# cmaestre/pcl_tracking

Hardware: AMD Instinct MI355X
Metric: particles x input-points / sec per frame (tracked frames/sec @8192 particles per GPU) (higher is better)
Workload: dtype f32

## Files before the change

pcl_tracking_amd/build.py:

```python
import os
import subprocess
import sys

_HERE = os.path.dirname(os.path.abspath(__file__))
CSRC = os.path.join(_HERE, "csrc")
OUT_DIR = os.path.join(_HERE, "_build")
LIB = os.path.join(OUT_DIR, "libpft_hip.so")
SOURCES = ["pft_kernels.hip", "pft_octree.hip", "pft_octree_gated.hip", "pft_octree_sorted.hip", "pft_likelihood.hip", "pft_population.hip", "pft_kld.hip", "pft_change.hip", "pft_exact_nn.hip", "pft_hull.hip", "pft_api.hip", "pft_frame.hip", "pft_api_debug.hip", "pft_api_features.hip",
           "pft_filters.hip", "pft_segment.hip", "pft_report.hip", "pft_model.hip", "pft_match.hip", "pft_reacquire.hip", "pft_spread.hip", "pft_refine.hip", "pft_subtract.hip", "pft_visibility.hip", "pft_depth.hip", "pft_grow.hip", "pft_view.hip"]
HEADERS = ["pft_internal.h", "pft_tracker.h", "pft_devbuf.h", "pft_device_utils.h", "pft_vis_project.h", "pft_alias.h", "pft_octree_box.h", "pft_report_solve.h", "pft_match_search.h", "pft_pair_tree.h", "pft_spread_final.h", "pft_refine_solve.h", "pft_segment_solve.h", os.path.join("..", "..", "include", "pft.h"),
           os.path.join("..", "..", "include", "pft_filters.h"), os.path.join("..", "..", "include", "pft_segment.h"),
           os.path.join("..", "..", "include", "pft_model.h"), os.path.join("..", "..", "include", "pft_subtract.h"),
           os.path.join("..", "..", "include", "pft_visibility.h"), os.path.join("..", "..", "include", "pft_grow.h"),
           os.path.join("..", "..", "include", "pft_view.h")]

HIPCC_FLAGS = [
    "--offload-arch=gfx950", "-O3", "-std=c++17", "-fPIC", "-shared", "-ffp-contract=off",
    "-fno-slp-vectorize",
    "-fno-fast-math", "-Wall", "-Wno-unused-function", "-Wno-unused-value", "-Wno-unused-result",
]


def hipcc():
    for c in (os.environ.get("HIPCC"), "/opt/rocm/bin/hipcc", "hipcc"):
        if c and (os.path.isabs(c) and os.path.exists(c) or not os.path.isabs(c)):
            return c
    return "hipcc"


def needs_build():
    if not os.path.exists(LIB):
        return True
    t = os.path.getmtime(LIB)
    deps = [os.path.join(CSRC, s) for s in SOURCES + HEADERS] + [os.path.abspath(__file__)]
    return any(os.path.getmtime(d) > t for d in deps)


def build(force=False, verbose=False, extra_flags=()):
    extra_flags = list(extra_flags) + os.environ.get("PFT_EXTRA_HIPCC_FLAGS", "").split()
    if not force and not needs_build():
        return LIB
    os.makedirs(OUT_DIR, exist_ok=True)
    cmd = [hipcc()] + HIPCC_FLAGS + list(extra_flags) + ["-o", LIB] + [os.path.join(CSRC, s) for s in SOURCES]
    if verbose:
        print(" ".join(cmd), flush=True)
    r = subprocess.run(cmd, capture_output=True, text=True)
    if r.returncode != 0:
        sys.stderr.write(r.stdout + r.stderr)
        raise RuntimeError("hipcc failed")
    if verbose and (r.stdout or r.stderr):
        print(r.stdout + r.stderr)
    return LIB


EXAMPLES_DIR = os.path.join(_HERE, "examples")
EXAMPLE_BIN = os.path.join(OUT_DIR, "auto_tracking_amd")
DIST_EXAMPLE_BIN = os.path.join(OUT_DIR, "dist_tracking_amd")
CREATE_MODEL_BIN = os.path.join(OUT_DIR, "create_model_amd")
_EXAMPLE_DEPS = [os.path.join(EXAMPLES_DIR, "tracking_app.hpp")] + [
    os.path.join(_HERE, "include", "pft", h) for h in ("particle_filter_tracker.hpp", "filters.hpp", "pcd_io.hpp", "common.hpp", "id_exchange.hpp", "segmentation.hpp", "model_preparation.hpp", "scene_subtraction.hpp", "model_growth.hpp", "pnm_io.hpp")] + [
    os.path.join(EXAMPLES_DIR, "segment_options.hpp")]


def _build_host_program(src, out, extra, force, verbose):
    lib = build()
    deps = [src, lib] + _EXAMPLE_DEPS
    if not force and os.path.exists(out) and all(os.path.getmtime(d) <= os.path.getmtime(out) for d in deps):
        return out
    root = os.path.dirname(_HERE)
    cmd = [hipcc(), "-std=c++17", "-O2", "-Wall", "-ffp-contract=off", "-I", os.path.join(root, "include"),
           "-I", os.path.join(_HERE, "include"), src, "-o", out, "-L", OUT_DIR, "-lpft_hip", "-Wl,-rpath,$ORIGIN"] + extra
    if verbose:
        print(" ".join(cmd), flush=True)
    r = subprocess.run(cmd, capture_output=True, text=True)
    if r.returncode != 0:
        sys.stderr.write(r.stdout + r.stderr)
        raise RuntimeError("example build failed: " + os.path.basename(src))
    return out


def build_host_program(src, out, force=False, verbose=False):
    return _build_host_program(src, out, [], force, verbose)


def build_example(force=False, verbose=False):
    return _build_host_program(os.path.join(EXAMPLES_DIR, "auto_tracking_amd.cpp"), EXAMPLE_BIN, [], force, verbose)


def build_dist_example(force=False, verbose=False):
    rocm = os.environ.get("ROCM_PATH", "/opt/rocm")
    extra = ["-I", os.path.join(rocm, "include"), "-L", os.path.join(rocm, "lib"), "-lrccl", "-lpthread",
             "-Wl,-rpath," + os.path.join(rocm, "lib")]
    return _build_host_program(os.path.join(EXAMPLES_DIR, "dist_tracking_amd.cpp"), DIST_EXAMPLE_BIN, extra, force, verbose)


def build_create_model_example(force=False, verbose=False):
    return _build_host_program(os.path.join(EXAMPLES_DIR, "create_model_amd.cpp"), CREATE_MODEL_BIN, [], force, verbose)


if __name__ == "__main__":
    print(build(force="--force" in sys.argv, verbose=True))
    print(build_example(force="--force" in sys.argv, verbose=True))
    print(build_dist_example(force="--force" in sys.argv, verbose=True))
    print(build_create_model_example(force="--force" in sys.argv, verbose=True))
```

pcl_tracking_amd/csrc/pft_octree.hip:

```cpp
#include "pft_device_utils.h"

#ifdef PFT_DIAG
#define STAMP(k) do { if (threadIdx.x == 0) d.hdr->ticks[k] = wall_clock64(); } while (0)
#define TICK_NOW() wall_clock64()
#else
#define STAMP(k) do { } while (0)
#define TICK_NOW() 0ull
#endif

#include "pft_octree_box.h"

#define PFT_REPLAY_HEAD 1024u
__device__ __forceinline__ void box_replay(BuildSh& S, const float4* __restrict__ pts, uint32_t n, double res, unsigned long long* hdr_ticks) {
  const uint32_t tid = threadIdx.x, nt = blockDim.x;
  const uint32_t head = n < PFT_REPLAY_HEAD ? n : PFT_REPLAY_HEAD;
  float lmn[3] = {FLT_MAX, FLT_MAX, FLT_MAX}, lmx[3] = {-FLT_MAX, -FLT_MAX, -FLT_MAX};
  const uint32_t wt = tid - WAVE, ws = nt - WAVE;
  auto local_aabb = [&]() {
    for (uint32_t i0 = PFT_REPLAY_HEAD + wt; i0 < n; i0 += 8u * ws) {
      float4 q[8];
#pragma unroll
      for (uint32_t k = 0; k < 8u; k++) q[k] = pts[min(i0 + k * ws, n - 1u)];
#pragma unroll
      for (uint32_t k = 0; k < 8u; k++) {
        lmn[0] = fminf(lmn[0], q[k].x); lmx[0] = fmaxf(lmx[0], q[k].x);
        lmn[1] = fminf(lmn[1], q[k].y); lmx[1] = fmaxf(lmx[1], q[k].y);
        lmn[2] = fminf(lmn[2], q[k].z); lmx[2] = fmaxf(lmx[2], q[k].z);
      }
    }
  };
  if (tid >= WAVE) local_aabb();
#ifdef PFT_DIAG
  if (tid == WAVE) hdr_ticks[13] = wall_clock64();
#endif
  if (tid < WAVE) {
    float4 q[PFT_REPLAY_HEAD / WAVE];
#pragma unroll
    for (uint32_t c = 0; c < PFT_REPLAY_HEAD / WAVE; c++) q[c] = pts[min(c * WAVE + tid, n - 1u)];
    uint32_t cur = 1;
    bool stop = false;
    double mn[3] = {S.mn[0], S.mn[1], S.mn[2]}, mx[3] = {S.mx[0], S.mx[1], S.mx[2]};
    int depth = S.depth, ngrow = S.ngrow;
    uint32_t err = S.err;
    const double epsd = (double)FLT_EPSILON;
#pragma unroll
    for (uint32_t c = 0; c < PFT_REPLAY_HEAD / WAVE; c++) {
      const uint32_t gi = c * WAVE + tid;
      const float4 p = q[c];
      while (!stop) {
        const bool viol = gi >= cur && gi < head && box_violates(p.x, p.y, p.z, mn, mx);
        const unsigned long long bal = __ballot(viol);
        if (!bal) break;
        const int f = __ffsll((long long)bal) - 1;
        const float px = __shfl(p.x, f), py = __shfl(p.y, f), pz = __shfl(p.z, f);
        const uint32_t idx = c * WAVE + (uint32_t)f;
        for (;;) {
          const bool lx = px < mn[0], ly = py < mn[1], lz = pz < mn[2];
          const bool ux = px >= mx[0], uy = py >= mx[1], uz = pz >= mx[2];
          if (!(lx || ly || lz || ux || uy || uz)) break;
          if (ngrow >= PFT_MAX_GROW || depth >= PFT_MAX_DEPTH) {
            err |= 2u;
            break;
          }
          double side = (double)(1u << depth) * res;
          if (tid == 0) {
            S.gidx[ngrow] = idx;
            S.gshift[ngrow] = (ux ? 0u : 1u) | (uy ? 0u : 2u) | (uz ? 0u : 4u);
            S.gold[ngrow] = (uint32_t)depth;
          }
          if (!ux) mn[0] -= side;
          if (!uy) mn[1] -= side;
          if (!uz) mn[2] -= side;
          depth++;
          side = (double)(1u << depth) * res - epsd;
          mx[0] = mn[0] + side;
          mx[1] = mn[1] + side;
          mx[2] = mn[2] + side;
          if (tid == 0) {
            S.gmin[ngrow + 1][0] = mn[0];
            S.gmin[ngrow + 1][1] = mn[1];
            S.gmin[ngrow + 1][2] = mn[2];
          }
          ngrow++;
        }
        cur = idx + 1u;
        if (err) stop = true;
      }
    }
    if (tid == 0) {
      for (int a = 0; a < 3; a++) {
        S.mn[a] = mn[a];
        S.mx[a] = mx[a];
      }
      S.depth = depth;
      S.ngrow = ngrow;
      S.err = err;
    }
    if (tid == 0) S.cur = head;
#ifdef PFT_DIAG
    if (tid == 0) hdr_ticks[14] = wall_clock64();
#endif
  }
  __syncthreads();
  if (S.err || n <= PFT_REPLAY_HEAD) return;
  for (;;) {
    const uint32_t cur = S.cur;
    const double mn[3] = {S.mn[0], S.mn[1], S.mn[2]};
    const double mx[3] = {S.mx[0], S.mx[1], S.mx[2]};
    uint32_t first = 0xffffffffu;
    if (tid >= WAVE && (box_violates(lmn[0], lmn[1], lmn[2], mn, mx) || box_violates(lmx[0], lmx[1], lmx[2], mn, mx))) {
      uint32_t i0 = PFT_REPLAY_HEAD + wt;
      if (i0 < cur) i0 += ((cur - i0 + ws - 1) / ws) * ws;
      for (uint32_t i = i0; i < n; i += ws) {
        const float4 p = pts[i];
        if (box_violates(p.x, p.y, p.z, mn, mx)) {
          first = i;
          break;
        }
      }
    }
    first = block_reduce<uint32_t>(first, S.u32s, OpMinU(), 0xffffffffu);
    if (first == 0xffffffffu) break;
    if (tid == 0) {
      box_grow(S, pts[first], first, res);
      S.cur = first + 1;
    }
    __syncthreads();
    if (S.err) break;
  }
}

template <int K>
struct RegStore {
  typedef uint32_t key_t;
  static constexpr int B = 10;
  static constexpr bool MORTON = true;
  static constexpr uint32_t CODE = K == 4 ? 1u : (K == 8 ? 2u : 3u);
  uint32_t key[K], node[K];
  __device__ RegStore(const PftDev&) {}
  template <class F>
  __device__ __forceinline__ void each(uint32_t n, F&& f) {
#pragma unroll
    for (int j = 0; j < K; j++) {
      uint32_t i = threadIdx.x + j * PFT_BUILD_THREADS;
      if (i < n) f(i, key[j], node[j]);
      UNROLL_FENCE(j, 2);
    }
  }
};

template <int K>
struct HybridStore {
  typedef uint32_t key_t;
  static constexpr int B = 10;
  static constexpr bool MORTON = true;
  static constexpr uint32_t CODE = 4u;
  uint32_t key[K], node[K];
  uint32_t* gkey;
  uint32_t* gnode;
  __device__ HybridStore(const PftDev& d) : gkey(reinterpret_cast<uint32_t*>(d.pt_key64)), gnode(d.pt_node) {}
  template <class F>
  __device__ __forceinline__ void each(uint32_t n, F&& f) {
#pragma unroll
    for (int j = 0; j < K; j++) {
      uint32_t i = threadIdx.x + j * PFT_BUILD_THREADS;
      if (i < n) f(i, key[j], node[j]);
      UNROLL_FENCE(j, 2);
    }
    for (uint32_t i = K * PFT_BUILD_THREADS + threadIdx.x; i < n; i += PFT_BUILD_THREADS) f(i, gkey[i], gnode[i]);
  }
};

struct GlobStore {
  typedef unsigned long long key_t;
  static constexpr int B = 21;
  static constexpr bool MORTON = false;
  static constexpr uint32_t CODE = 5u;
  unsigned long long* key;
  uint32_t* node;
  __device__ GlobStore(const PftDev& d) : key(d.pt_key64), node(d.pt_node) {}
  template <class F>
  __device__ __forceinline__ void each(uint32_t n, F&& f) {
#pragma unroll 4
    for (uint32_t i = threadIdx.x; i < n; i += blockDim.x) f(i, key[i], node[i]);
  }
};

template <class KT, int B, bool MORTON>
__device__ __forceinline__ uint32_t key_child(KT k, int bit) {
  if (MORTON) return (uint32_t)(k >> (3 * bit)) & 7u;
  return (uint32_t)(((k >> (2 * B + bit)) & 1) << 2) | (uint32_t)(((k >> (B + bit)) & 1) << 1) |
         (uint32_t)((k >> bit) & 1);
}

__device__ __forceinline__ uint32_t spread3_10(uint32_t x) {
  x = (x | (x << 16)) & 0x030000FFu;
  x = (x | (x << 8)) & 0x0300F00Fu;
  x = (x | (x << 4)) & 0x030C30C3u;
  x = (x | (x << 2)) & 0x09249249u;
  return x;
}

template <class Store, bool LDSW, bool TMPLDS>
__device__ __forceinline__ bool build_tree(const PftParams& prm, const PftDev& d, BuildSh& S, uint32_t n, uint32_t* lds_words,
                           uint32_t lds_words_cap, uint32_t* lds_tmp, uint32_t* out_leaf_start,
                           uint32_t* out_n_leaves) {
  typedef typename Store::key_t key_t;
  constexpr int B = Store::B;
  const uint32_t tid = threadIdx.x, nt = blockDim.x;
  const float4* pts = d.crop_pts;
  const double res = prm.res, inv_res = 1.0 / prm.res;
  const int D = S.depth, ngrow = S.ngrow;
  Store st(d);
  const int J = (D >= 4 && D <= PFT_TABLE_MAX_DEPTH) ? (D - 1 < PFT_JUMP_MAX_LEVEL ? D - 1 : PFT_JUMP_MAX_LEVEL) : 0;
  if (J > 0) {
    for (uint32_t i = tid; i < 128u; i += nt) S.dn_bits[J][i] = 0u;
    __syncthreads();
  }

  const uint32_t last_grow = ngrow > 0 ? S.gidx[ngrow - 1] : 0u;
  st.each(n, [&](uint32_t i, key_t& key, uint32_t& node) {
    float4 p = pts[i];
    int e = ngrow;
    if (ngrow > 0 && i < last_grow) {
      e = 0;
      while (e < ngrow && S.gidx[e] <= i) e++;
    }
    const double tq[3] = {(double)p.x - S.gmin[e][0], (double)p.y - S.gmin[e][1], (double)p.z - S.gmin[e][2]};
    uint32_t kk[3];
#pragma unroll
    for (int a = 0; a < 3; a++) {
      double q0 = tq[a] * inv_res;
      const double fr = q0 - floor(q0);
      if (fr < 1.0e-6 || fr > 1.0 - 1.0e-6) q0 = tq[a] / res;
      kk[a] = (uint32_t)q0;
    }
    uint32_t kx = kk[0], ky = kk[1], kz = kk[2];
    for (int s = e; s < ngrow; s++) {
      uint32_t sh = S.gshift[s], od = S.gold[s];
      if (sh & 1u) kx += 1u << od;
      if (sh & 2u) ky += 1u << od;
      if (sh & 4u) kz += 1u << od;
    }
    if (d.pt_key) {
      d.pt_key[3 * (size_t)i + 0] = kx;
      d.pt_key[3 * (size_t)i + 1] = ky;
      d.pt_key[3 * (size_t)i + 2] = kz;
    }
    if (Store::MORTON)
      key = (key_t)((spread3_10(kx) << 2) | (spread3_10(ky) << 1) | spread3_10(kz));
    else
      key = ((key_t)kx << (2 * B)) | ((key_t)ky << B) | (key_t)kz;
    node = 0;
  });

  STAMP(2);
  uint32_t* W = LDSW ? lds_words : d.words;
  if (tid == 0) S.jump = J;
  int l0 = 0;
  if (J > 0) {
    uint32_t (*dn_bits)[128] = S.dn_bits;
    uint32_t (*dn_pref)[128] = S.dn_pref;
    uint32_t* dn_cnt = S.dn_cnt;
    st.each(n, [&](uint32_t, key_t& key, uint32_t& node) {
      uint32_t mj = 0;
      if (Store::MORTON)
        mj = (uint32_t)(key >> (3 * (D - J)));
      else
        for (int l = 0; l < J; l++) mj = (mj << 3) | key_child<key_t, B, Store::MORTON>(key, D - 1 - l);
      node = mj;
      const uint32_t bt = 1u << (mj & 31u);
      if (!(dn_bits[J][mj >> 5] & bt)) atomicOr(&dn_bits[J][mj >> 5], bt);
    });
    __syncthreads();
    for (int l = J - 1; l >= 0; l--) {
      const uint32_t nbits = 1u << (3 * l);
      const bool pred = tid < nbits && ((dn_bits[l + 1][tid >> 2] >> (8u * (tid & 3u))) & 0xffu) != 0u;
      const unsigned long long m = __ballot(pred);
      if (lane_id() == 0 && (uint32_t)wave_id() * 64u < ((nbits + 63u) & ~63u)) {
        dn_bits[l][2 * wave_id()] = (uint32_t)m;
        dn_bits[l][2 * wave_id() + 1] = (uint32_t)(m >> 32);
      }
      __syncthreads();
    }
    if (wave_id() <= J) {
      const int l = wave_id(), ln = lane_id();
      const uint32_t nwords = ((1u << (3 * l)) + 31u) >> 5;
      const uint32_t c0 = (uint32_t)ln < nwords ? __popc(dn_bits[l][ln]) : 0u;
      const uint32_t c1 = (uint32_t)ln + 64u < nwords ? __popc(dn_bits[l][ln + 64]) : 0u;
      const uint32_t i0 = wave_incl_scan(c0);
      const uint32_t t0 = (uint32_t)__shfl((int)i0, 63);
      const uint32_t i1 = wave_incl_scan(c1);
      dn_pref[l][ln] = i0 - c0;
      dn_pref[l][ln + 64] = t0 + i1 - c1;
      if (ln == 63) dn_cnt[l] = t0 + i1;
    }
    __syncthreads();
    if (tid == 0) {
      S.lvl[0] = 0;
      for (int l = 0; l <= J; l++) S.lvl[l + 1] = S.lvl[l] + dn_cnt[l];
    }
    __syncthreads();
    const uint32_t top_end = S.lvl[J + 1];
    if (LDSW && top_end + 2 > lds_words_cap) return false;
    if (top_end + 2 > d.max_words) {
      if (tid == 0) S.err |= 1u;
    } else {
#define DN_RANK(l, i) (dn_pref[l][(i) >> 5] + __popc(dn_bits[l][(i) >> 5] & ((1u << ((i) & 31u)) - 1u)))
      for (uint32_t cand = tid; cand < 585u; cand += nt) {
        int l = 0;
        uint32_t i = cand;
        while (l < J && i >= (1u << (3 * l))) {
          i -= 1u << (3 * l);
          l++;
        }
        if (l < J && ((dn_bits[l][i >> 5] >> (i & 31u)) & 1u)) {
          const uint32_t mask = (dn_bits[l + 1][i >> 2] >> (8u * (i & 3u))) & 0xffu;
          const uint32_t base = S.lvl[l + 1] + DN_RANK(l + 1, 8u * i);
          W[S.lvl[l] + DN_RANK(l, i)] = mask | (base << 8);
        }
      }
      for (uint32_t j = S.lvl[J] + tid; j < top_end; j += nt) W[j] = 0;
      for (uint32_t i = tid; i < (1u << (3 * J)); i += nt) {
        uint32_t cx = 0, cy = 0, cz = 0;
        for (int b = 0; b < J; b++) {
          const uint32_t dg = (i >> (3 * b)) & 7u;
          cx |= (dg >> 2) << b;
          cy |= ((dg >> 1) & 1u) << b;
          cz |= (dg & 1u) << b;
        }
        const bool occ = (dn_bits[J][i >> 5] >> (i & 31u)) & 1u;
        d.jump[cx | (cy << J) | (cz << (2 * J))] = occ ? (uint16_t)(DN_RANK(J, i) + 1u) : (uint16_t)0;
      }
      const uint32_t lj = S.lvl[J];
      st.each(n, [&](uint32_t, key_t&, uint32_t& node) { node = lj + DN_RANK(J, node); });
#undef DN_RANK
    }
    __syncthreads();
    l0 = J;
  } else {
    if (tid == 0) {
      W[0] = 0;
      S.lvl[0] = 0;
      S.lvl[1] = 1;
    }
    __syncthreads();
  }

  unsigned long long tA = 0, tB = 0, tC = 0, tD = 0, t0_, t1_;
  for (int l = l0; l < D && !S.err; l++) {
    const int bit = D - 1 - l;
    t0_ = TICK_NOW();
    st.each(n, [&](uint32_t, key_t& key, uint32_t& node) {
      if (l > l0) {
        uint32_t w = W[node];
        uint32_t cp = key_child<key_t, B, Store::MORTON>(key, bit + 1);
        node = (w >> 8) + __popc(w & 0xffu & ((1u << cp) - 1u));
      }
      const uint32_t cb = 1u << key_child<key_t, B, Store::MORTON>(key, bit);
      if (!(W[node] & cb)) atomicOr(&W[node], cb);
    });
    __syncthreads();
    t1_ = TICK_NOW(); tA += t1_ - t0_; t0_ = t1_;
    const uint32_t ls = S.lvl[l], le = S.lvl[l + 1], nl = le - ls;
    const uint32_t per = (nl + nt - 1) / nt;
    const uint32_t a0 = ls + min(nl, tid * per), a1 = ls + min(nl, (tid + 1) * per);
    uint32_t cnt = 0;
    for (uint32_t nd = a0; nd < a1; nd++) cnt += __popc(W[nd] & 0xffu);
    t1_ = TICK_NOW(); tB += t1_ - t0_; t0_ = t1_;
    uint32_t* scr = S.u32s + (l & 1) * 20;
    uint32_t inc = wave_incl_scan(cnt);
    if (lane_id() == WAVE - 1) scr[wave_id()] = inc;
    __syncthreads();
    if (wave_id() == 0) {
      const int nw = (int)(nt >> 6);
      uint32_t t = lane_id() < nw ? scr[lane_id()] : 0u;
      uint32_t ti = wave_incl_scan(t);
      if (lane_id() < nw) scr[lane_id()] = ti - t;
      if (lane_id() == nw - 1) scr[17] = ti;
    }
    __syncthreads();
    t1_ = TICK_NOW(); tC += t1_ - t0_; t0_ = t1_;
    uint32_t base = le + scr[wave_id()] + inc - cnt;
    const uint32_t nend = le + scr[17];
    const bool overflow = nend + 2 > d.max_words || nend >= (1u << 24);
    if (LDSW && !overflow && nend + 2 > lds_words_cap) return false;
    if (overflow) {
      if (tid == 0) S.err |= 1u;
    } else {
      for (uint32_t nd = a0; nd < a1; nd++) {
        const uint32_t wv = W[nd];
        W[nd] = wv | (base << 8);
        base += __popc(wv & 0xffu);
      }
      for (uint32_t j = le + tid; j < nend; j += nt) W[j] = 0;
    }
    if (tid == 0) S.lvl[l + 2] = nend;
    __syncthreads();
    t1_ = TICK_NOW(); tD += t1_ - t0_;
    if (S.err) break;
  }
#ifdef PFT_DIAG
  if (tid == 0) { d.hdr->ticks[9] = tA; d.hdr->ticks[10] = tB; d.hdr->ticks[11] = tC; d.hdr->ticks[12] = tD; }
#endif
  __syncthreads();
  if (S.err || D <= 0) {
    *out_leaf_start = 0;
    *out_n_leaves = 0;
    return true;
  }

  STAMP(3);
  const uint32_t leaf_start = S.lvl[D], n_leaves = S.lvl[D + 1] - leaf_start;
  st.each(n, [&](uint32_t, key_t& key, uint32_t& node) {
    uint32_t w = W[node];
    uint32_t c = key_child<key_t, B, Store::MORTON>(key, 0);
    uint32_t leaf = (w >> 8) + __popc(w & 0xffu & ((1u << c) - 1u));
    node = leaf;
    key = (key_t)atomicAdd(&W[leaf], 1u);
  });
  __syncthreads();
  {
    const uint32_t per = (n_leaves + nt - 1) / nt;
    const uint32_t a0 = leaf_start + min(n_leaves, tid * per), a1 = leaf_start + min(n_leaves, (tid + 1) * per);
    uint32_t cnt = 0;
    for (uint32_t nd = a0; nd < a1; nd++) cnt += W[nd];
    uint32_t total;
    uint32_t start = block_excl_scan<uint32_t>(cnt, S.u32s, &total);
    for (uint32_t nd = a0; nd < a1; nd++) {
      const uint32_t c = W[nd];
      W[nd] = start;
      start += c;
    }
  }
  if (tid == 0) {
    W[leaf_start + n_leaves] = n;
    S.variant = Store::CODE | (LDSW ? 8u : 0u) | (TMPLDS ? 16u : 0u);
  }
  __syncthreads();
  STAMP(4);
  uint32_t* TMP = TMPLDS ? lds_tmp : d.pt_tmp;
  st.each(n, [&](uint32_t i, key_t& key, uint32_t& node) { TMP[W[node] + (uint32_t)key] = i; });
  __syncthreads();
  STAMP(5);
  st.each(n, [&](uint32_t i, key_t&, uint32_t& node) {
    const uint32_t s = W[node], e = W[node + 1];
    uint32_t rank = 0;
    for (uint32_t k = s; k < e; k++) rank += TMP[k] < i ? 1u : 0u;
    d.leaf_order[s + rank] = i;
  });
  STAMP(6);
  const uint32_t n_words = leaf_start + n_leaves + 1;
  if (LDSW)
    for (uint32_t j = tid; j < n_words; j += nt) d.words[j] = W[j];
  *out_leaf_start = leaf_start;
  *out_n_leaves = n_leaves;
  return true;
}

template <class Store>
__device__ __forceinline__ void build_tree_any(const PftParams& prm, const PftDev& d, BuildSh& S, uint32_t n,
                                               uint32_t* lds_words, uint32_t cap, uint32_t* lds_tmp, uint32_t* ls,
                                               uint32_t* nl) {
  bool done = false;
  if (cap >= 64) {
    if (lds_tmp) done = build_tree<Store, true, true>(prm, d, S, n, lds_words, cap, lds_tmp, ls, nl);
    else done = build_tree<Store, true, false>(prm, d, S, n, lds_words, cap, lds_tmp, ls, nl);
  }
  __syncthreads();
  if (!done) build_tree<Store, false, false>(prm, d, S, n, lds_words, cap, lds_tmp, ls, nl);
}

template <int K>
__device__ __forceinline__ void build_hybrid(const PftParams& prm, const PftDev& d, BuildSh& S, uint32_t n, uint32_t* lds_words,
                             uint32_t cap, uint32_t* lds_tmp, uint32_t* ls, uint32_t* nl, int* path) {
  if (S.depth <= HybridStore<K>::B) {
    *path = 2;
    build_tree_any<HybridStore<K>>(prm, d, S, n, lds_words, cap, lds_tmp, ls, nl);
  } else {
    build_tree_any<GlobStore>(prm, d, S, n, lds_words, cap, lds_tmp, ls, nl);
  }
}

template <int K>
__device__ __forceinline__ void build_regs(const PftParams& prm, const PftDev& d, BuildSh& S, uint32_t n, uint32_t* lds_words,
                           uint32_t cap, uint32_t* lds_tmp, uint32_t* ls, uint32_t* nl, int* path) {
  if (S.depth <= RegStore<K>::B) {
    *path = 1;
    build_tree_any<RegStore<K>>(prm, d, S, n, lds_words, cap, lds_tmp, ls, nl);
  } else {
    build_tree_any<GlobStore>(prm, d, S, n, lds_words, cap, lds_tmp, ls, nl);
  }
}

template <bool GATED>
__global__ __launch_bounds__(PFT_BUILD_THREADS) void k_octree_build(PftParams prm, PftDev d, uint32_t lds_bytes,
                                                                    int copy_leaf_pts, int rescue, int anc_up) {
  extern __shared__ __attribute__((aligned(16))) unsigned char smem[];
  __shared__ BuildSh S;
  PftHeader* hdr = d.hdr;
  if (rescue && !(hdr->error & 8u)) return;
  const uint32_t tid = threadIdx.x;
  const float4 p_first = tid == 0 ? d.crop_pts[0] : make_float4(0, 0, 0, 0);
  const uint32_t n = hdr->n_crop;
  if (GATED && pft_unchanged(d.gate)) return;

  STAMP(0);
  if (tid == 0) {
    S.err = hdr->error & 4u;
    S.ngrow = 0;
    S.depth = 0;
    S.cur = 1;
    S.variant = 0;
    if (n > 0) box_init(S, p_first, prm.res);
  }
  __syncthreads();

  uint32_t* lds_u = reinterpret_cast<uint32_t*>(smem);
  const uint32_t lds_words_total = lds_bytes / 4u;
  uint32_t* lds_tmp = nullptr;
  uint32_t tmp_words = 0;
  if ((size_t)n * 5u / 2u + 64u <= lds_words_total) {
    lds_tmp = lds_u;
    tmp_words = (n + 3u) & ~3u;
  }
  uint32_t* lds_words = lds_u + tmp_words;
  const uint32_t cap = lds_words_total - tmp_words;

  uint32_t leaf_start = 0, n_leaves = 0;
  int path = 0;
  if (n > 0) {
    box_replay(S, d.crop_pts, n, prm.res, d.hdr->ticks);
    __syncthreads();
    STAMP(1);
  }
  if (n > 0 && !S.err) {
    if (n <= 4u * PFT_BUILD_THREADS) build_regs<4>(prm, d, S, n, lds_words, cap, lds_tmp, &leaf_start, &n_leaves, &path);
    else if (n <= 8u * PFT_BUILD_THREADS) build_regs<8>(prm, d, S, n, lds_words, cap, lds_tmp, &leaf_start, &n_leaves, &path);
    else if (n <= 14u * PFT_BUILD_THREADS) build_regs<14>(prm, d, S, n, lds_words, cap, lds_tmp, &leaf_start, &n_leaves, &path);
    else if (n <= 18u * PFT_BUILD_THREADS) build_hybrid<8>(prm, d, S, n, lds_words, cap, lds_tmp, &leaf_start, &n_leaves, &path);
    else build_tree_any<GlobStore>(prm, d, S, n, lds_words, cap, lds_tmp, &leaf_start, &n_leaves);
  }
  __syncthreads();
  STAMP(7);
  const int D = S.depth;
  const bool ok = n > 0 && !S.err && D > 0;
  if (copy_leaf_pts == 1 && ok) {
    __threadfence_block();
    for (uint32_t pos = tid; pos < n; pos += blockDim.x) d.leaf_pts[pos] = d.crop_pts[d.leaf_order[pos]];
  }

  const int use_table = (ok && D <= PFT_TABLE_MAX_DEPTH) ? 1 : 0;
  STAMP(8);
  if (tid == 0) {
    hdr->error = S.err;
    hdr->depth = D;
    hdr->use_table = use_table;
    hdr->n_grow = S.ngrow;
    hdr->build_path = path;
    const uint32_t lds_total = lds_bytes / 4u, var = S.variant;
    const bool tried = lds_total - ((size_t)n * 5u / 2u + 64u <= lds_total ? ((n + 3u) & ~3u) : 0u) >= 64u;
    hdr->build_variant = var | ((var && !(var & 8u) && tried) ? 32u : 0u) | ((ok && use_table && S.jump > 0) ? 64u : 0u) |
                         (rescue ? 128u : 0u) | ((uint32_t)copy_leaf_pts << 8);
    hdr->leaf_indirect = copy_leaf_pts == 2 ? 1 : 0;
    if (d.host_stat) d.host_stat[1] = (uint32_t)D;
    hdr->jump_level = (ok && use_table) ? S.jump : 0;
    hdr->n_leaves = ok ? n_leaves : 0;
    hdr->leaf_start = ok ? leaf_start : 0;
    hdr->n_words = ok ? leaf_start + n_leaves + 1 : 0;
  }
  if (tid == 64) {
    double maxabs = 0.0;
    for (int a = 0; a < 3; a++) maxabs = fmax(maxabs, fmax(fabs(S.mn[a]), fabs(S.mx[a])));
    const double eta = maxabs * 1.1920928955078125e-07;
    const double s_top = prm.res * (double)(1u << (D > 0 ? D - 1 : 0));
    const double E = 9.0 * eta + 40.0 * 5.9604644775390625e-08 * s_top;
    double mc = 2.0 * E / prm.res + 1.0e-3;
    hdr->margin_cells = (float)(mc < 0.25 ? mc : 1.0);
  }
  if (tid == 128) hdr->inv_res = (float)(1.0 / prm.res);
  if (tid == 320) pft_anc_window(hdr, d, D, ok && use_table, copy_leaf_pts == 0, S.mn, prm.res, anc_up);
  if (tid >= 192 && tid < 195) {
    const int a = (int)tid - 192;
    hdr->ominf[a] = (float)S.mn[a];
    hdr->omin[a] = n > 0 ? S.mn[a] : 0.0;
    hdr->omax[a] = n > 0 ? S.mx[a] : 0.0;
  }
  if (tid >= 256 && tid < 256 + PFT_MAX_DEPTH + 3 && (int)tid - 256 <= D + 1) hdr->lvl_start[tid - 256] = S.lvl[tid - 256];
}

__device__ __forceinline__ void anc_fill(const PftDev& d, uint32_t gid, uint32_t stride) {
  const PftHeader* hdr = d.hdr;
  const int L = hdr->anc_level;
  if (L <= 0) return;
  const bool deeper = hdr->depth - L == 1;
  const int Lw = deeper ? L - 1 : L;
  const uint32_t bx = hdr->anc_bits[0], by = hdr->anc_bits[1], bz = hdr->anc_bits[2];
  const uint32_t wbx = deeper ? bx - 1u : bx, wby = deeper ? by - 1u : by, wbz = deeper ? bz - 1u : bz;
  const uint32_t n = 1u << (wbx + wby + wbz);
  const uint32_t x0 = hdr->anc_lo[0] >> (deeper ? 1 : 0), y0 = hdr->anc_lo[1] >> (deeper ? 1 : 0),
                 z0 = hdr->anc_lo[2] >> (deeper ? 1 : 0);
  const int J = hdr->jump_level <= Lw ? hdr->jump_level : 0;
  const uint32_t lvlJ = J > 0 ? hdr->lvl_start[J] : 0u;
  for (uint32_t c = gid; c < n; c += stride) {
    const uint32_t ux = c & ((1u << wbx) - 1u), uy = (c >> wbx) & ((1u << wby) - 1u), uz = c >> (wbx + wby);
    const uint32_t x = x0 + ux, y = y0 + uy, z = z0 + uz;
    uint32_t node = 0;
    int lvl = 0;
    if (J > 0) {
      const int sh = Lw - J;
      const uint32_t e = d.jump[(x >> sh) | ((y >> sh) << J) | ((z >> sh) << (2 * J))];
      node = e ? lvlJ + e - 1u : 0u;
      lvl = e ? J : 0;
    }
    for (; lvl < Lw; lvl++) {
      const int sh = Lw - lvl - 1;
      const uint32_t ch = (((x >> sh) & 1u) << 2) | (((y >> sh) & 1u) << 1) | ((z >> sh) & 1u);
      const uint32_t wv = d.words[node];
      if (!((wv >> ch) & 1u)) break;
      node = (wv >> 8) + __popc(wv & 0xffu & ((1u << ch) - 1u));
    }
    const uint32_t own = ((uint32_t)lvl << 27) | node;
    if (!deeper) {
      d.anc[c] = own;
    } else {
      const uint32_t wv = lvl == Lw ? d.words[node] : 0u;
      const uint32_t mask = wv & 0xffu, base = wv >> 8;
#pragma unroll
      for (uint32_t yz = 0; yz < 4u; yz++) {
        const uint32_t c0 = yz, c1 = 4u | yz;
        uint2 e;
        e.x = (mask >> c0) & 1u ? ((uint32_t)L << 27) | (base + __popc(mask & ((1u << c0) - 1u))) : own;
        e.y = (mask >> c1) & 1u ? ((uint32_t)L << 27) | (base + __popc(mask & ((1u << c1) - 1u))) : own;
        const uint32_t idx = (2u * ux) | ((2u * uy + (yz >> 1)) << bx) | ((2u * uz + (yz & 1u)) << (bx + by));
        *reinterpret_cast<uint2*>(d.anc + idx) = e;
      }
    }
  }
  if (gid == 0) d.hdr->anc_epoch = hdr->build_epoch;
}

template <bool GATED>
__global__ __launch_bounds__(256) void k_leaf_gather(PftDev d) {
  if (GATED && pft_unchanged(d.gate)) return;
  const PftHeader* hdr = d.hdr;
  const uint32_t pos = blockIdx.x * 256u + threadIdx.x;
  if (hdr->error || hdr->depth <= 0) return;
  if (pos < hdr->n_crop) d.leaf_pts[pos] = d.crop_pts[d.leaf_order[pos]];
  anc_fill(d, pos, gridDim.x * 256u);
}

#ifndef PFT_OCTREE_GATED_TU
extern template __global__ void k_octree_build<true>(PftParams, PftDev, uint32_t, int, int, int);
extern template __global__ void k_leaf_gather<true>(PftDev);

static void pftk_octree_set_attr() {
  static bool attr_set[PFT_MAX_DEVICES];
  const uint32_t lds = ((uint32_t)pftk_max_lds_bytes() - 10240u) & ~15u;
  const int dev = pftk_cur_device();
  if (!attr_set[dev])
    attr_set[dev] = hipFuncSetAttribute(reinterpret_cast<const void*>(&k_octree_build<false>),
                                        hipFuncAttributeMaxDynamicSharedMemorySize, (int)lds) == hipSuccess &&
                    hipFuncSetAttribute(reinterpret_cast<const void*>(&k_octree_build<true>),
                                        hipFuncAttributeMaxDynamicSharedMemorySize, (int)lds) == hipSuccess;
}

void pftk_octree(hipStream_t s, const PftParams& p, const PftDev& d, uint32_t expected_points, bool indirect, int anc_up) {
  const uint32_t lds = ((uint32_t)pftk_max_lds_bytes() - 10240u) & ~15u;
  pftk_octree_set_attr();
  const int mode = indirect ? 2 : (expected_points <= PFT_GATHER_MIN ? 1 : 0);
  const dim3 gg((d.N + 255u) / 256u ? (d.N + 255u) / 256u : 1u);
  if (d.gate) {
    hipLaunchKernelGGL(k_octree_build<true>, dim3(1), dim3(PFT_BUILD_THREADS), lds, s, p, d, lds, mode, 0, anc_up);
    if (mode == 0) hipLaunchKernelGGL(k_leaf_gather<true>, gg, dim3(256), 0, s, d);
  } else {
    hipLaunchKernelGGL(k_octree_build<false>, dim3(1), dim3(PFT_BUILD_THREADS), lds, s, p, d, lds, mode, 0, anc_up);
    if (mode == 0) hipLaunchKernelGGL(k_leaf_gather<false>, gg, dim3(256), 0, s, d);
  }
}

void pftk_octree_rescue(hipStream_t s, const PftParams& p, const PftDev& d) {
  pftk_octree_set_attr();
  const uint32_t lds = ((uint32_t)pftk_max_lds_bytes() - 10240u) & ~15u;
  if (d.gate)
    hipLaunchKernelGGL(k_octree_build<true>, dim3(1), dim3(PFT_BUILD_THREADS), lds, s, p, d, lds, 1, 1, 0);
  else
    hipLaunchKernelGGL(k_octree_build<false>, dim3(1), dim3(PFT_BUILD_THREADS), lds, s, p, d, lds, 1, 1, 0);
}
#endif
```

Baseline: 879.1 billion.

## Prefetch points into registers during box replay and overlap LDS zeroing

During the serial wave-0 box replay, the other waves now prefetch the crop points into registers, fold their AABB, and zero the LDS tree words and jump bitmaps ahead of time. The register-resident build path then computes keys from these preloaded coordinates instead of reloading them from global memory. Box bounds are precomputed as rounded-up floats so violation checks avoid double compares. Level offsets are computed per thread from the counts, removing a serial step and a barrier. This adds register pressure and a more complex fallback path that must re-zero the jump bitmaps.

```diff
diff --git a/pcl_tracking_amd/build.py b/pcl_tracking_amd/build.py
--- a/pcl_tracking_amd/build.py
+++ b/pcl_tracking_amd/build.py
@@ -8,7 +8,7 @@
 LIB = os.path.join(OUT_DIR, "libpft_hip.so")
 SOURCES = ["pft_kernels.hip", "pft_octree.hip", "pft_octree_gated.hip", "pft_octree_sorted.hip", "pft_likelihood.hip", "pft_population.hip", "pft_kld.hip", "pft_change.hip", "pft_exact_nn.hip", "pft_hull.hip", "pft_api.hip", "pft_frame.hip", "pft_api_debug.hip", "pft_api_features.hip",
            "pft_filters.hip", "pft_segment.hip", "pft_report.hip", "pft_model.hip", "pft_match.hip", "pft_reacquire.hip", "pft_spread.hip", "pft_refine.hip", "pft_subtract.hip", "pft_visibility.hip", "pft_depth.hip", "pft_grow.hip", "pft_view.hip"]
-HEADERS = ["pft_internal.h", "pft_tracker.h", "pft_devbuf.h", "pft_device_utils.h", "pft_vis_project.h", "pft_alias.h", "pft_octree_box.h", "pft_report_solve.h", "pft_match_search.h", "pft_pair_tree.h", "pft_spread_final.h", "pft_refine_solve.h", "pft_segment_solve.h", os.path.join("..", "..", "include", "pft.h"),
+HEADERS = ["pft_internal.h", "pft_tracker.h", "pft_devbuf.h", "pft_device_utils.h", "pft_vis_project.h", "pft_alias.h", "pft_octree_box.h", "pft_box_bounds.h", "pft_report_solve.h", "pft_match_search.h", "pft_pair_tree.h", "pft_spread_final.h", "pft_refine_solve.h", "pft_segment_solve.h", os.path.join("..", "..", "include", "pft.h"),
            os.path.join("..", "..", "include", "pft_filters.h"), os.path.join("..", "..", "include", "pft_segment.h"),
            os.path.join("..", "..", "include", "pft_model.h"), os.path.join("..", "..", "include", "pft_subtract.h"),
            os.path.join("..", "..", "include", "pft_visibility.h"), os.path.join("..", "..", "include", "pft_grow.h"),
diff --git a/pcl_tracking_amd/csrc/pft_box_bounds.h b/pcl_tracking_amd/csrc/pft_box_bounds.h
--- /dev/null
+++ b/pcl_tracking_amd/csrc/pft_box_bounds.h
@@ -0,0 +1,37 @@
+#pragma once
+#include <float.h>
+#include <math.h>
+
+#if defined(__HIPCC__)
+#define PFT_BB_HD __device__ __forceinline__
+#else
+#define PFT_BB_HD inline
+#endif
+
+PFT_BB_HD float box_bound_ru(double b) {
+  if (b != b) return (float)b;
+  if (b == 0.0) return 0.0f;
+  if (b > (double)FLT_MAX) return (float)INFINITY;
+  if (b == -(double)INFINITY) return -(float)INFINITY;
+  if (b < -(double)FLT_MAX) return -FLT_MAX;
+  float f = (float)b;
+  if ((double)f < b) f = nextafterf(f, (float)INFINITY);
+  return f;
+}
+
+struct BoxBoundsF {
+  float lo[3], hi[3];
+};
+
+PFT_BB_HD BoxBoundsF box_bounds_f(const double* mn, const double* mx) {
+  BoxBoundsF b;
+  for (int a = 0; a < 3; a++) {
+    b.lo[a] = box_bound_ru(mn[a]);
+    b.hi[a] = box_bound_ru(mx[a]);
+  }
+  return b;
+}
+
+PFT_BB_HD bool box_violates_f(float x, float y, float z, const BoxBoundsF& b) {
+  return (x < b.lo[0]) || (y < b.lo[1]) || (z < b.lo[2]) || (x >= b.hi[0]) || (y >= b.hi[1]) || (z >= b.hi[2]);
+}
diff --git a/pcl_tracking_amd/csrc/pft_octree.hip b/pcl_tracking_amd/csrc/pft_octree.hip
--- a/pcl_tracking_amd/csrc/pft_octree.hip
+++ b/pcl_tracking_amd/csrc/pft_octree.hip
@@ -9,13 +9,39 @@
 #endif
 
 #include "pft_octree_box.h"
+#include "pft_box_bounds.h"
 
 #define PFT_REPLAY_HEAD 1024u
-__device__ __forceinline__ void box_replay(BuildSh& S, const float4* __restrict__ pts, uint32_t n, double res, unsigned long long* hdr_ticks) {
+#define PFT_PRE_K 8
+struct PrePts {
+  float x[PFT_PRE_K], y[PFT_PRE_K], z[PFT_PRE_K];
+};
+__device__ __forceinline__ void pre_load(PrePts& pre, const float4* __restrict__ pts, uint32_t n, int j0) {
+#pragma unroll
+  for (int j = j0; j < PFT_PRE_K; j++) {
+    if ((uint32_t)j * PFT_BUILD_THREADS < n) {
+      const float4 q = pts[min(threadIdx.x + (uint32_t)j * PFT_BUILD_THREADS, n - 1u)];
+      pre.x[j] = q.x;
+      pre.y[j] = q.y;
+      pre.z[j] = q.z;
+    }
+  }
+}
+
+__device__ __forceinline__ void box_replay(BuildSh& S, BoxBoundsF& Sbf, const float4* __restrict__ pts, uint32_t n, double res,
+                                           unsigned long long* hdr_ticks, uint32_t* lds_zero, uint32_t zero_words, PrePts& pre) {
   const uint32_t tid = threadIdx.x, nt = blockDim.x;
   const uint32_t head = n < PFT_REPLAY_HEAD ? n : PFT_REPLAY_HEAD;
+  const bool use_pre = n <= PFT_PRE_K * PFT_BUILD_THREADS;
   float lmn[3] = {FLT_MAX, FLT_MAX, FLT_MAX}, lmx[3] = {-FLT_MAX, -FLT_MAX, -FLT_MAX};
   const uint32_t wt = tid - WAVE, ws = nt - WAVE;
+  float ex = 0.0f, ey = 0.0f, ez = 0.0f;
+  uint32_t ei = 0xffffffffu;
+  auto fold = [&](float x, float y, float z) {
+    lmn[0] = fminf(lmn[0], x); lmx[0] = fmaxf(lmx[0], x);
+    lmn[1] = fminf(lmn[1], y); lmx[1] = fmaxf(lmx[1], y);
+    lmn[2] = fminf(lmn[2], z); lmx[2] = fmaxf(lmx[2], z);
+  };
   auto local_aabb = [&]() {
     for (uint32_t i0 = PFT_REPLAY_HEAD + wt; i0 < n; i0 += 8u * ws) {
       float4 q[8];
@@ -29,17 +55,40 @@
       }
     }
   };
-  if (tid >= WAVE) local_aabb();
+  const bool wave0 = __builtin_amdgcn_readfirstlane((int)(tid >> 6)) == 0;
+  if (!wave0) {
+    if (use_pre) {
+      pre_load(pre, pts, n, 0);
+      if (wt < (PFT_PRE_K - 1) * WAVE) {
+        const uint32_t i = (wt & (WAVE - 1u)) + (1u + wt / WAVE) * PFT_BUILD_THREADS;
+        if (i < n) {
+          const float4 q = pts[i];
+          ex = q.x, ey = q.y, ez = q.z;
+          ei = i;
+          fold(ex, ey, ez);
+        }
+      }
+#pragma unroll
+      for (int j = 1; j < PFT_PRE_K; j++)
+        if ((uint32_t)j * PFT_BUILD_THREADS < n) fold(pre.x[j], pre.y[j], pre.z[j]);
+    } else {
+      local_aabb();
+    }
+    uint32_t* dnb = &S.dn_bits[0][0];
+    for (uint32_t i = wt; i < (PFT_JUMP_MAX_LEVEL + 1) * 128u; i += ws) dnb[i] = 0u;
+    uint4* z4 = reinterpret_cast<uint4*>(lds_zero);
+    for (uint32_t i = wt; i < zero_words / 4u; i += ws) z4[i] = make_uint4(0u, 0u, 0u, 0u);
 #ifdef PFT_DIAG
-  if (tid == WAVE) hdr_ticks[13] = wall_clock64();
+    if (tid == WAVE) hdr_ticks[13] = wall_clock64();
 #endif
-  if (tid < WAVE) {
+  } else {
     float4 q[PFT_REPLAY_HEAD / WAVE];
 #pragma unroll
     for (uint32_t c = 0; c < PFT_REPLAY_HEAD / WAVE; c++) q[c] = pts[min(c * WAVE + tid, n - 1u)];
     uint32_t cur = 1;
     bool stop = false;
     double mn[3] = {S.mn[0], S.mn[1], S.mn[2]}, mx[3] = {S.mx[0], S.mx[1], S.mx[2]};
+    BoxBoundsF bf = box_bounds_f(mn, mx);
     int depth = S.depth, ngrow = S.ngrow;
     uint32_t err = S.err;
     const double epsd = (double)FLT_EPSILON;
@@ -48,7 +97,7 @@
       const uint32_t gi = c * WAVE + tid;
       const float4 p = q[c];
       while (!stop) {
-        const bool viol = gi >= cur && gi < head && box_violates(p.x, p.y, p.z, mn, mx);
+        const bool viol = gi >= cur && gi < head && box_violates_f(p.x, p.y, p.z, bf);
         const unsigned long long bal = __ballot(viol);
         if (!bal) break;
         const int f = __ffsll((long long)bal) - 1;
@@ -83,9 +132,16 @@
           }
           ngrow++;
         }
+        bf = box_bounds_f(mn, mx);
         cur = idx + 1u;
         if (err) stop = true;
       }
+    }
+    if (use_pre) {
+      pre.x[0] = q[0].x;
+      pre.y[0] = q[0].y;
+      pre.z[0] = q[0].z;
+      pre_load(pre, pts, n, 1);
     }
     if (tid == 0) {
       for (int a = 0; a < 3; a++) {
@@ -95,6 +151,7 @@
       S.depth = depth;
       S.ngrow = ngrow;
       S.err = err;
+      Sbf = bf;
     }
     if (tid == 0) S.cur = head;
 #ifdef PFT_DIAG
@@ -105,17 +162,25 @@
   if (S.err || n <= PFT_REPLAY_HEAD) return;
   for (;;) {
     const uint32_t cur = S.cur;
-    const double mn[3] = {S.mn[0], S.mn[1], S.mn[2]};
-    const double mx[3] = {S.mx[0], S.mx[1], S.mx[2]};
+    const BoxBoundsF bf = Sbf;
     uint32_t first = 0xffffffffu;
-    if (tid >= WAVE && (box_violates(lmn[0], lmn[1], lmn[2], mn, mx) || box_violates(lmx[0], lmx[1], lmx[2], mn, mx))) {
-      uint32_t i0 = PFT_REPLAY_HEAD + wt;
-      if (i0 < cur) i0 += ((cur - i0 + ws - 1) / ws) * ws;
-      for (uint32_t i = i0; i < n; i += ws) {
-        const float4 p = pts[i];
-        if (box_violates(p.x, p.y, p.z, mn, mx)) {
-          first = i;
-          break;
+    if (tid >= WAVE && (box_violates_f(lmn[0], lmn[1], lmn[2], bf) || box_violates_f(lmx[0], lmx[1], lmx[2], bf))) {
+      if (use_pre) {
+        if (ei < n && ei >= cur && box_violates_f(ex, ey, ez, bf)) first = ei;
+#pragma unroll
+        for (int j = PFT_PRE_K - 1; j >= 1; j--) {
+          const uint32_t i = tid + (uint32_t)j * PFT_BUILD_THREADS;
+          if (i >= cur && i < n && box_violates_f(pre.x[j], pre.y[j], pre.z[j], bf)) first = min(first, i);
+        }
+      } else {
+        uint32_t i0 = PFT_REPLAY_HEAD + wt;
+        if (i0 < cur) i0 += ((cur - i0 + ws - 1) / ws) * ws;
+        for (uint32_t i = i0; i < n; i += ws) {
+          const float4 p = pts[i];
+          if (box_violates_f(p.x, p.y, p.z, bf)) {
+            first = i;
+            break;
+          }
         }
       }
     }
@@ -124,6 +189,7 @@
     if (tid == 0) {
       box_grow(S, pts[first], first, res);
       S.cur = first + 1;
+      Sbf = box_bounds_f(S.mn, S.mx);
     }
     __syncthreads();
     if (S.err) break;
@@ -138,6 +204,15 @@
   static constexpr uint32_t CODE = K == 4 ? 1u : (K == 8 ? 2u : 3u);
   uint32_t key[K], node[K];
   __device__ RegStore(const PftDev&) {}
+  template <class F>
+  __device__ __forceinline__ void each_j(uint32_t n, F&& f) {
+#pragma unroll
+    for (int j = 0; j < K; j++) {
+      uint32_t i = threadIdx.x + j * PFT_BUILD_THREADS;
+      if (i < n) f(i, j, key[j], node[j]);
+      UNROLL_FENCE(j, 2);
+    }
+  }
   template <class F>
   __device__ __forceinline__ void each(uint32_t n, F&& f) {
 #pragma unroll
@@ -201,10 +276,10 @@
   return x;
 }
 
-template <class Store, bool LDSW, bool TMPLDS>
+template <class Store, bool LDSW, bool TMPLDS, bool PRE>
 __device__ __forceinline__ bool build_tree(const PftParams& prm, const PftDev& d, BuildSh& S, uint32_t n, uint32_t* lds_words,
-                           uint32_t lds_words_cap, uint32_t* lds_tmp, uint32_t* out_leaf_start,
-                           uint32_t* out_n_leaves) {
+                           uint32_t lds_words_cap, uint32_t lds_zeroed, uint32_t* lds_tmp, uint32_t* out_leaf_start,
+                           uint32_t* out_n_leaves, const PrePts& pre) {
   typedef typename Store::key_t key_t;
   constexpr int B = Store::B;
   const uint32_t tid = threadIdx.x, nt = blockDim.x;
@@ -213,20 +288,16 @@
   const int D = S.depth, ngrow = S.ngrow;
   Store st(d);
   const int J = (D >= 4 && D <= PFT_TABLE_MAX_DEPTH) ? (D - 1 < PFT_JUMP_MAX_LEVEL ? D - 1 : PFT_JUMP_MAX_LEVEL) : 0;
-  if (J > 0) {
-    for (uint32_t i = tid; i < 128u; i += nt) S.dn_bits[J][i] = 0u;
-    __syncthreads();
-  }
+  const uint32_t zeroed = LDSW ? lds_zeroed : 0u;
 
   const uint32_t last_grow = ngrow > 0 ? S.gidx[ngrow - 1] : 0u;
-  st.each(n, [&](uint32_t i, key_t& key, uint32_t& node) {
-    float4 p = pts[i];
+  auto key_of = [&](uint32_t i, float px, float py, float pz, key_t& key, uint32_t& node) {
     int e = ngrow;
     if (ngrow > 0 && i < last_grow) {
       e = 0;
       while (e < ngrow && S.gidx[e] <= i) e++;
     }
-    const double tq[3] = {(double)p.x - S.gmin[e][0], (double)p.y - S.gmin[e][1], (double)p.z - S.gmin[e][2]};
+    const double tq[3] = {(double)px - S.gmin[e][0], (double)py - S.gmin[e][1], (double)pz - S.gmin[e][2]};
     uint32_t kk[3];
 #pragma unroll
     for (int a = 0; a < 3; a++) {
@@ -252,7 +323,19 @@
     else
       key = ((key_t)kx << (2 * B)) | ((key_t)ky << B) | (key_t)kz;
     node = 0;
-  });
+  };
+  if constexpr (PRE) {
+    st.each_j(n, [&](uint32_t i, int j, key_t& key, uint32_t& node) {
+      float px = pre.x[j], py = pre.y[j], pz = pre.z[j];
+      asm volatile("" : "+v"(px), "+v"(py), "+v"(pz));
+      key_of(i, px, py, pz, key, node);
+    });
+  } else {
+    st.each(n, [&](uint32_t i, key_t& key, uint32_t& node) {
+      const float4 p = pts[i];
+      key_of(i, p.x, p.y, p.z, key, node);
+    });
+  }
 
   STAMP(2);
   uint32_t* W = LDSW ? lds_words : d.words;
@@ -296,12 +379,20 @@
       if (ln == 63) dn_cnt[l] = t0 + i1;
     }
     __syncthreads();
-    if (tid == 0) {
-      S.lvl[0] = 0;
-      for (int l = 0; l <= J; l++) S.lvl[l + 1] = S.lvl[l] + dn_cnt[l];
-    }
-    __syncthreads();
-    const uint32_t top_end = S.lvl[J + 1];
+    uint32_t cnt_l[PFT_JUMP_MAX_LEVEL + 1];
+#pragma unroll
+    for (int k = 0; k <= PFT_JUMP_MAX_LEVEL; k++) {
+      const uint32_t c = dn_cnt[k];
+      cnt_l[k] = k <= J ? c : 0u;
+    }
+    auto lvl_at = [&](int l) {
+      uint32_t r = 0;
+#pragma unroll
+      for (int k = 0; k <= PFT_JUMP_MAX_LEVEL; k++) r += k < l ? cnt_l[k] : 0u;
+      return r;
+    };
+    if (tid <= (uint32_t)J + 1u) S.lvl[tid] = lvl_at((int)tid);
+    const uint32_t top_end = lvl_at(J + 1);
     if (LDSW && top_end + 2 > lds_words_cap) return false;
     if (top_end + 2 > d.max_words) {
       if (tid == 0) S.err |= 1u;
@@ -316,11 +407,11 @@
         }
         if (l < J && ((dn_bits[l][i >> 5] >> (i & 31u)) & 1u)) {
           const uint32_t mask = (dn_bits[l + 1][i >> 2] >> (8u * (i & 3u))) & 0xffu;
-          const uint32_t base = S.lvl[l + 1] + DN_RANK(l + 1, 8u * i);
-          W[S.lvl[l] + DN_RANK(l, i)] = mask | (base << 8);
+          const uint32_t base = lvl_at(l + 1) + DN_RANK(l + 1, 8u * i);
+          W[lvl_at(l) + DN_RANK(l, i)] = mask | (base << 8);
         }
       }
-      for (uint32_t j = S.lvl[J] + tid; j < top_end; j += nt) W[j] = 0;
+      for (uint32_t j = max(lvl_at(J), zeroed) + tid; j < top_end; j += nt) W[j] = 0;
       for (uint32_t i = tid; i < (1u << (3 * J)); i += nt) {
         uint32_t cx = 0, cy = 0, cz = 0;
         for (int b = 0; b < J; b++) {
@@ -332,7 +423,7 @@
         const bool occ = (dn_bits[J][i >> 5] >> (i & 31u)) & 1u;
         d.jump[cx | (cy << J) | (cz << (2 * J))] = occ ? (uint16_t)(DN_RANK(J, i) + 1u) : (uint16_t)0;
       }
-      const uint32_t lj = S.lvl[J];
+      const uint32_t lj = lvl_at(J);
       st.each(n, [&](uint32_t, key_t&, uint32_t& node) { node = lj + DN_RANK(J, node); });
 #undef DN_RANK
     }
@@ -393,7 +484,7 @@
         W[nd] = wv | (base << 8);
         base += __popc(wv & 0xffu);
       }
-      for (uint32_t j = le + tid; j < nend; j += nt) W[j] = 0;
+      for (uint32_t j = max(le, zeroed) + tid; j < nend; j += nt) W[j] = 0;
     }
     if (tid == 0) S.lvl[l + 2] = nend;
     __syncthreads();
@@ -458,38 +549,43 @@
   return true;
 }
 
-template <class Store>
+template <class Store, bool PRE>
 __device__ __forceinline__ void build_tree_any(const PftParams& prm, const PftDev& d, BuildSh& S, uint32_t n,
-                                               uint32_t* lds_words, uint32_t cap, uint32_t* lds_tmp, uint32_t* ls,
-                                               uint32_t* nl) {
+                                               uint32_t* lds_words, uint32_t cap, uint32_t zw, uint32_t* lds_tmp, uint32_t* ls,
+                                               uint32_t* nl, const PrePts& pre) {
   bool done = false;
   if (cap >= 64) {
-    if (lds_tmp) done = build_tree<Store, true, true>(prm, d, S, n, lds_words, cap, lds_tmp, ls, nl);
-    else done = build_tree<Store, true, false>(prm, d, S, n, lds_words, cap, lds_tmp, ls, nl);
+    if (lds_tmp) done = build_tree<Store, true, true, PRE>(prm, d, S, n, lds_words, cap, zw, lds_tmp, ls, nl, pre);
+    else done = build_tree<Store, true, false, PRE>(prm, d, S, n, lds_words, cap, zw, lds_tmp, ls, nl, pre);
+    if (!done) {
+      __syncthreads();
+      uint32_t* dnb = &S.dn_bits[0][0];
+      for (uint32_t i = threadIdx.x; i < (PFT_JUMP_MAX_LEVEL + 1) * 128u; i += blockDim.x) dnb[i] = 0u;
+    }
   }
   __syncthreads();
-  if (!done) build_tree<Store, false, false>(prm, d, S, n, lds_words, cap, lds_tmp, ls, nl);
+  if (!done) build_tree<Store, false, false, false>(prm, d, S, n, lds_words, cap, 0u, lds_tmp, ls, nl, pre);
 }
 
 template <int K>
 __device__ __forceinline__ void build_hybrid(const PftParams& prm, const PftDev& d, BuildSh& S, uint32_t n, uint32_t* lds_words,
-                             uint32_t cap, uint32_t* lds_tmp, uint32_t* ls, uint32_t* nl, int* path) {
+                             uint32_t cap, uint32_t zw, uint32_t* lds_tmp, uint32_t* ls, uint32_t* nl, int* path, const PrePts& pre) {
   if (S.depth <= HybridStore<K>::B) {
     *path = 2;
-    build_tree_any<HybridStore<K>>(prm, d, S, n, lds_words, cap, lds_tmp, ls, nl);
+    build_tree_any<HybridStore<K>, false>(prm, d, S, n, lds_words, cap, zw, lds_tmp, ls, nl, pre);
   } else {
-    build_tree_any<GlobStore>(prm, d, S, n, lds_words, cap, lds_tmp, ls, nl);
+    build_tree_any<GlobStore, false>(prm, d, S, n, lds_words, cap, zw, lds_tmp, ls, nl, pre);
   }
 }
 
 template <int K>
 __device__ __forceinline__ void build_regs(const PftParams& prm, const PftDev& d, BuildSh& S, uint32_t n, uint32_t* lds_words,
-                           uint32_t cap, uint32_t* lds_tmp, uint32_t* ls, uint32_t* nl, int* path) {
+                           uint32_t cap, uint32_t zw, uint32_t* lds_tmp, uint32_t* ls, uint32_t* nl, int* path, const PrePts& pre) {
   if (S.depth <= RegStore<K>::B) {
     *path = 1;
-    build_tree_any<RegStore<K>>(prm, d, S, n, lds_words, cap, lds_tmp, ls, nl);
+    build_tree_any<RegStore<K>, (K <= PFT_PRE_K)>(prm, d, S, n, lds_words, cap, zw, lds_tmp, ls, nl, pre);
   } else {
-    build_tree_any<GlobStore>(prm, d, S, n, lds_words, cap, lds_tmp, ls, nl);
+    build_tree_any<GlobStore, false>(prm, d, S, n, lds_words, cap, zw, lds_tmp, ls, nl, pre);
   }
 }
 
@@ -498,11 +594,12 @@
                                                                     int copy_leaf_pts, int rescue, int anc_up) {
   extern __shared__ __attribute__((aligned(16))) unsigned char smem[];
   __shared__ BuildSh S;
+  __shared__ BoxBoundsF Sbf;
   PftHeader* hdr = d.hdr;
   if (rescue && !(hdr->error & 8u)) return;
   const uint32_t tid = threadIdx.x;
   const float4 p_first = tid == 0 ? d.crop_pts[0] : make_float4(0, 0, 0, 0);
-  const uint32_t n = hdr->n_crop;
+  const uint32_t n = (uint32_t)__builtin_amdgcn_readfirstlane((int)hdr->n_crop);
   if (GATED && pft_unchanged(d.gate)) return;
 
   STAMP(0);
@@ -526,20 +623,22 @@
   }
   uint32_t* lds_words = lds_u + tmp_words;
   const uint32_t cap = lds_words_total - tmp_words;
+  const uint32_t zw = cap >= 64u ? min(cap, (2u * n + 67u) & ~3u) : 0u;
 
   uint32_t leaf_start = 0, n_leaves = 0;
   int path = 0;
+  PrePts pre;
   if (n > 0) {
-    box_replay(S, d.crop_pts, n, prm.res, d.hdr->ticks);
+    box_replay(S, Sbf, d.crop_pts, n, prm.res, d.hdr->ticks, lds_words, zw, pre);
     __syncthreads();
     STAMP(1);
   }
   if (n > 0 && !S.err) {
-    if (n <= 4u * PFT_BUILD_THREADS) build_regs<4>(prm, d, S, n, lds_words, cap, lds_tmp, &leaf_start, &n_leaves, &path);
-    else if (n <= 8u * PFT_BUILD_THREADS) build_regs<8>(prm, d, S, n, lds_words, cap, lds_tmp, &leaf_start, &n_leaves, &path);
-    else if (n <= 14u * PFT_BUILD_THREADS) build_regs<14>(prm, d, S, n, lds_words, cap, lds_tmp, &leaf_start, &n_leaves, &path);
-    else if (n <= 18u * PFT_BUILD_THREADS) build_hybrid<8>(prm, d, S, n, lds_words, cap, lds_tmp, &leaf_start, &n_leaves, &path);
-    else build_tree_any<GlobStore>(prm, d, S, n, lds_words, cap, lds_tmp, &leaf_start, &n_leaves);
+    if (n <= 4u * PFT_BUILD_THREADS) build_regs<4>(prm, d, S, n, lds_words, cap, zw, lds_tmp, &leaf_start, &n_leaves, &path, pre);
+    else if (n <= 8u * PFT_BUILD_THREADS) build_regs<8>(prm, d, S, n, lds_words, cap, zw, lds_tmp, &leaf_start, &n_leaves, &path, pre);
+    else if (n <= 14u * PFT_BUILD_THREADS) build_regs<14>(prm, d, S, n, lds_words, cap, zw, lds_tmp, &leaf_start, &n_leaves, &path, pre);
+    else if (n <= 18u * PFT_BUILD_THREADS) build_hybrid<8>(prm, d, S, n, lds_words, cap, zw, lds_tmp, &leaf_start, &n_leaves, &path, pre);
+    else build_tree_any<GlobStore, false>(prm, d, S, n, lds_words, cap, zw, lds_tmp, &leaf_start, &n_leaves, pre);
   }
   __syncthreads();
   STAMP(7);
```

After: 855.5 billion. -2.7%, worse.
